# BVE-Reborn/rend3

Measured on NVIDIA H100. Metric: culled objects/s (fused frustum cull + object-uniform bake), higher is better.
Workload: dtype f32

## Files before the change

rend3_b200/csrc/r3_common.cuh:

```cuda
#pragma once
#include <cuda_runtime.h>
#include <stdint.h>

#include <string>
#include <vector>

#include "../../include/rend3_b200.h"

#define R3_EXPORT extern "C" __attribute__((visibility("default")))

constexpr int R3_MAX_CAMERAS = 64;

struct r3_iobuf {
    uint8_t* d = nullptr;
    uint64_t capacity_elements = 0, out_elems = 0, in_elems = 0, elem_size = 0;
    bool flipped = false, clear_on_swap = false, created = false;
    uint64_t out_off() const { return flipped ? capacity_elements / 2 : 0; }
    uint64_t in_off() const { return flipped ? 0 : capacity_elements / 2; }
};

struct r3_jobs {
    r3_batch_data* d_batches = nullptr; uint32_t batches_cap = 0, n_batches = 0;
    r3_region* d_regions = nullptr; uint32_t regions_cap = 0, n_regions = 0;
    uint32_t* d_region_first_inv = nullptr;
// ... 58 lines not shown
struct r3_anim_state;

struct r3_tri_record { float xyw[3][3]; uint32_t object_id; uint32_t vid[3]; uint32_t _pad[3]; };
static_assert(sizeof(r3_tri_record) == 64, "triangle record");

struct r3_ctx {
    int device = 0;
    cudaStream_t stream = nullptr;
    cudaStream_t side_stream = nullptr;
    std::string err;
    uint64_t launches = 0;
    bool coop_launch_ok = false;
    int sm_count = 1;
    r3_object* d_objects = nullptr; uint32_t n_slots = 0, objects_cap = 0; bool objects_borrowed = false;
    float4* d_hot_xyz = nullptr; float4* d_hot_w = nullptr; float4* d_hot_sphere = nullptr; uint32_t* d_enabled_bits = nullptr; uint32_t* d_affine_bits = nullptr;
    uint64_t hot_cap = 0; bool hot_valid = false;
    std::vector<uint64_t> sort_key; std::vector<uint8_t> sort_flags; std::vector<float> sort_loc;
    uint32_t* d_live_bits = nullptr; uint32_t live_bits_cap = 0; bool have_live = false;
    uint8_t* d_sort_key8 = nullptr; float* d_sort_loc = nullptr; uint32_t sort_dev_cap = 0; bool gpu_batching_ok = false;
    float4* d_mesh_spheres = nullptr; uint32_t n_mesh_spheres = 0, mesh_spheres_cap = 0;
    bool locations_moved = false;
    uint32_t sort_live_blend = 0, sort_wide_keys = 0;
    unsigned long long* d_gsort_keys[2] = {nullptr, nullptr}; uint64_t gsort_cap[2] = {0, 0}; uint32_t* d_gsort_hist = nullptr; uint64_t gsort_hist_cap = 0;
    uint32_t* d_gsort_header = nullptr; int gsort_src = 0; uint32_t gsort_n = 0; bool gsort_valid = false; float gsort_loc[3] = {0, 0, 0};
    uint64_t gsort_epoch = 0, gsort_sorted_epoch = ~0ull; uint32_t gsort_cameras_this_epoch = 0, gsort_cameras_last_epoch = 0;
    uint64_t max_total_invocations = 0, max_object_invocations = 0; bool max_invocations_valid = false;
    uint32_t* d_mesh = nullptr; uint64_t mesh_words = 0, mesh_cap = 0;
    r3_material* d_materials = nullptr; uint32_t n_materials = 0, materials_cap = 0;
    bool has_skybox = false; r3_texture_desc sky_desc{}; uint8_t* d_sky_texels = nullptr; uint64_t sky_cap = 0;
    r3_texture_desc* d_tex_descs = nullptr; uint32_t n_textures = 0, tex_descs_cap = 0; uint8_t* d_texels = nullptr; uint64_t texels_cap = 0, texel_bytes = 0;
// ... 67 lines not shown
template <typename T, typename C>
int r3_reserve_t(r3_ctx* c, T** ptr, C* cap, uint64_t need, bool keep = false, bool zero_new = false) {
    uint64_t cap64 = *cap;
    int rc = r3_reserve(c, (void**)ptr, &cap64, need, sizeof(T), keep, zero_new);
    *cap = (C)cap64;
    return rc;
}

int r3_launch_cull_bake(r3_ctx* c, r3_camera* cam, uint32_t mode);
int r3_launch_cull_bake_device_camera(r3_ctx* c, r3_camera* cam, uint32_t mode, const r3_camera_header* d_header);
int r3_camera_buffers(r3_ctx* c, r3_camera* cam, uint32_t mode);
int r3_split_objects(r3_ctx* c);
int r3_split_slots(r3_ctx* c, const uint32_t* d_slots, uint32_t n);
int r3_grow_hot(r3_ctx* c, uint32_t old_n, uint32_t n);
uint64_t r3_hot_capacity(uint64_t want);
int r3_launch_mask_word(r3_ctx* c, uint32_t* word_a, uint32_t* word_b, uint32_t keep_mask);
int r3_launch_triangle_cull(r3_ctx* c, r3_camera* cam);
int r3_host_batch_objects(r3_ctx* c, r3_camera* cam, const float vp_loc[3], uint32_t max_dispatch_count);
int r3_upload_jobs(r3_ctx* c, r3_camera* cam);
int r3_device_batch_objects(r3_ctx* c, r3_camera* cam, const float vp_loc[3], uint32_t max_dispatch_count);
int r3_download_jobs(r3_ctx* c, r3_camera* cam);
int r3_compute_max_invocations(r3_ctx* c);
void r3_new_frame_epoch(r3_ctx* c);
int r3_blend_collect(r3_ctx* c, bool* ran);
int r3_iobuf_new(r3_ctx* c, r3_iobuf* b, uint64_t elems, uint64_t elem_size, bool clear_on_swap);
int r3_iobuf_swap(r3_ctx* c, r3_iobuf* b, uint64_t new_elems);
int r3_launch_skinning(r3_ctx* c, const r3_skinning_input* d_inputs, const uint32_t* d_chunk_prefix, uint32_t n_skeletons, uint32_t total_chunks,
                       const float* d_joints, uint32_t n_joints);
void r3_anim_destroy(r3_ctx* c);
int r3_anim_stage_posed_locations(r3_ctx* c, bool* staged);
void r3_anim_apply_posed_locations(r3_ctx* c);
int r3_stage_moved_locations(r3_ctx* c, bool* staged);
int r3_grow_mesh_spheres(r3_ctx* c, uint32_t n);
int r3_reserve_point_buffer(r3_ctx* c, uint32_t n_lights);

#ifdef __CUDACC__
__device__ __forceinline__ uint32_t affine_w_bits(uint32_t j) { return j == 3 ? 0x3f800000u : 0u; }
__device__ __forceinline__ float mul_rn(float a, float b) { return __fmul_rn(a, b); }
__device__ __forceinline__ float add_rn(float a, float b) { return __fadd_rn(a, b); }
__device__ __forceinline__ float sub_rn(float a, float b) { return __fsub_rn(a, b); }
__device__ __forceinline__ float div_rn(float a, float b) { return __fdiv_rn(a, b); }
__device__ __forceinline__ float4 mat_vec_rn(const float* __restrict__ m, float x, float y, float z, float w) {
    float4 r;
    r.x = mul_rn(m[0], x); r.y = mul_rn(m[1], x); r.z = mul_rn(m[2], x); r.w = mul_rn(m[3], x);
    r.x = add_rn(r.x, mul_rn(m[4], y)); r.y = add_rn(r.y, mul_rn(m[5], y)); r.z = add_rn(r.z, mul_rn(m[6], y)); r.w = add_rn(r.w, mul_rn(m[7], y));
    r.x = add_rn(r.x, mul_rn(m[8], z)); r.y = add_rn(r.y, mul_rn(m[9], z)); r.z = add_rn(r.z, mul_rn(m[10], z)); r.w = add_rn(r.w, mul_rn(m[11], z));
    r.x = add_rn(r.x, mul_rn(m[12], w)); r.y = add_rn(r.y, mul_rn(m[13], w)); r.z = add_rn(r.z, mul_rn(m[14], w)); r.w = add_rn(r.w, mul_rn(m[15], w));
    return r;
}
__device__ __forceinline__ float4 mat_point_rn(const float* __restrict__ m, float x, float y, float z) {
    float4 r;
    r.x = mul_rn(m[0], x); r.y = mul_rn(m[1], x); r.z = mul_rn(m[2], x); r.w = mul_rn(m[3], x);
// ... 7 lines not shown
```

rend3_b200/csrc/r3_ctx.cu:

```cuda
#include <algorithm>
#include <cstdio>
#include <cstdlib>
#include <cstring>
#include <new>

#include "r3_common.cuh"

int r3_fail(r3_ctx* c, int code, const char* msg) {
    if (c) c->err = msg;
    return code;
}
int r3_cuda_fail(r3_ctx* c, cudaError_t e, const char* where) {
    if (c) {
        c->err = std::string(where) + ": " + cudaGetErrorString(e);
    }
    cudaGetLastError();
    return e == cudaErrorMemoryAllocation ? R3_E_OOM : R3_E_CUDA;
}

int r3_reserve(r3_ctx* c, void** ptr, uint64_t* cap, uint64_t need, size_t elem, bool keep, bool zero_new) {
    if (*ptr && *cap >= need) return R3_OK;
    uint64_t ncap = need < 16 ? 16 : need;
    void* n = nullptr;
    R3_CUDA(c, cudaMalloc(&n, ncap * elem));
// ... 38 lines not shown
    cudaMemsetAsync(c->d_point, 0, c->point_bytes_cap, c->stream);
    *out = c;
    return R3_OK;
}

static void free_jobs(r3_jobs& j) { cudaFree(j.d_batches); cudaFree(j.d_regions); cudaFree(j.d_region_first_inv); cudaFree(j.d_header); }

R3_EXPORT int r3_ctx_destroy(r3_ctx* c) {
    if (!c) return R3_E_INVALID;
    cudaSetDevice(c->device);
    r3_stream_sync(c);
    if (c->side_stream) cudaStreamSynchronize(c->side_stream);
    r3_peer_destroy(c);
    r3_anim_destroy(c);
    if (!c->objects_borrowed) cudaFree(c->d_objects);
    cudaFree(c->d_hot_xyz); cudaFree(c->d_hot_w); cudaFree(c->d_hot_sphere); cudaFree(c->d_enabled_bits); cudaFree(c->d_affine_bits); cudaFree(c->d_tex_descs); cudaFree(c->d_texels); cudaFree(c->d_sky_texels);
    cudaFree(c->d_sort_key8); cudaFree(c->d_sort_loc); cudaFree(c->d_gsort_keys[0]); cudaFree(c->d_gsort_keys[1]); cudaFree(c->d_gsort_hist); cudaFree(c->d_gsort_header);
    cudaFree(c->d_mesh_spheres); cudaFree(c->d_live_bits); cudaFree(c->d_mesh); cudaFree(c->d_materials); cudaFree(c->d_dir); cudaFree(c->d_point);
    cudaFree(c->d_light_mats); cudaFree(c->d_atlas); cudaFree(c->d_light_src); cudaFree(c->d_shadow_cams); cudaFree(c->d_point_src); cudaFree(c->d_point_live);
    for (auto& k : c->cams) {
        cudaFree(k.d_matrices); cudaFree(k.d_visible); cudaFree(k.d_visible_count); cudaFree(k.d_tile_state);
        if (k.d_gathered) {
            for (uint32_t r = 0; r < k.ex_ranks; ++r)
                if (k.ex_connected && r != k.ex_rank && k.ex_peers[r]) cudaIpcCloseMemHandle(k.ex_peers[r]);
            cudaFree(k.d_gathered);
        }
        cudaFree(k.d_ex_done); cudaFree(k.d_global_visible); cudaFree(k.d_merge_counts);
        for (int q = 0; q < R3_EXCHANGE_SLOTS; ++q) { if (k.ex_cull_done[q]) cudaEventDestroy(k.ex_cull_done[q]); if (k.ex_merge_done[q]) cudaEventDestroy(k.ex_merge_done[q]); }
        free_jobs(k.jobs[0]); free_jobs(k.jobs[1]);
        cudaFree(k.index_buffer.d); cudaFree(k.draw_call_buffer.d); cudaFree(k.results_buffer.d);
        cudaFree(k.d_resid_bits); cudaFree(k.d_word_scan); cudaFree(k.d_block_sums);
// ... 401 lines not shown
    if (n == c->n_slots) return R3_OK;
    cudaSetDevice(c->device);
    const uint32_t old_n = c->n_slots;
    if (n > c->objects_cap || !c->d_objects) R3_TRY(r3_reserve_t(c, &c->d_objects, &c->objects_cap, r3_hot_capacity(n), true));
    R3_CUDA(c, cudaMemsetAsync(c->d_objects + old_n, 0, (size_t)(n - old_n) * sizeof(r3_object), c->stream));
    R3_TRY(r3_grow_hot(c, old_n, n));
    R3_TRY(r3_grow_mesh_spheres(c, n));
    c->n_slots = n;
    const size_t sorted = c->sort_key.size();
    if (c->have_live && sorted < n) {
        c->sort_key.resize(n, 0); c->sort_flags.resize(n, 0); c->sort_loc.resize(3 * (size_t)n, 0.0f);
        const uint32_t old_words = (uint32_t)((sorted + 31) / 32), words = (n + 31) / 32;
        R3_TRY(r3_reserve_t(c, &c->d_live_bits, &c->live_bits_cap, words, true));
        const uint32_t whole = (sorted & 31u) ? old_words : (uint32_t)(sorted / 32);
        if (words > whole) R3_CUDA(c, cudaMemsetAsync(c->d_live_bits + whole, 0, (size_t)(words - whole) * 4, c->stream));
        if (sorted & 31u) R3_TRY(r3_launch_mask_word(c, c->d_live_bits + sorted / 32, nullptr, (1u << (sorted & 31u)) - 1u));
        if (n > c->sort_dev_cap || !c->d_sort_key8) {
            const uint32_t cap = (uint32_t)r3_hot_capacity(n);
            uint8_t* k8 = nullptr; float* l = nullptr;
            R3_CUDA(c, cudaMalloc((void**)&k8, cap));
            R3_CUDA(c, cudaMalloc((void**)&l, ((size_t)cap * 3 + 4) * 4));
            if (sorted) {
                R3_CUDA(c, cudaMemcpyAsync(k8, c->d_sort_key8, sorted, cudaMemcpyDeviceToDevice, c->stream));
                R3_CUDA(c, cudaMemcpyAsync(l, c->d_sort_loc, sorted * 12, cudaMemcpyDeviceToDevice, c->stream));
            }
            R3_CUDA(c, r3_stream_sync(c));
            cudaFree(c->d_sort_key8); cudaFree(c->d_sort_loc);
            c->d_sort_key8 = k8; c->d_sort_loc = l; c->sort_dev_cap = cap;
        }
        R3_CUDA(c, cudaMemsetAsync(c->d_sort_key8 + sorted, 0, n - sorted, c->stream));
        R3_CUDA(c, cudaMemsetAsync(c->d_sort_loc + 3 * sorted, 0, (n - sorted) * 12, c->stream));
// ... 290 lines not shown
```

rend3_b200/csrc/r3_cull_bake.cu:

```cuda
#include <cstdlib>
#include <type_traits>

#include "r3_common.cuh"
#include "r3_scan.cuh"

namespace {

constexpr int CB_THREADS = 256;
constexpr int CB_WARPS = CB_THREADS / 32;
constexpr int CB_WT = 4;
constexpr int CB_CTA_OBJECTS = CB_WARPS * CB_WT * 32;
constexpr int CP_THREADS = 1024;
constexpr int CP_OBJECTS = CP_THREADS * 32;
constexpr int CP_CTAS_PER_TILE = CP_OBJECTS / CB_CTA_OBJECTS;

struct CullBakeParams {
    float view[16];
    float view_proj[16];
    float frustum[5][4];
    uint32_t object_count;
};
struct DeviceCameraParams {
    const r3_camera_header* cam;
    uint32_t object_count;
};
constexpr int CAM_FLOATS = 52;

__global__ void __launch_bounds__(256) split_objects_kernel(const float4* __restrict__ objects, uint32_t n, float* __restrict__ rows_xyz, float* __restrict__ rows_w,
                                                            float4* __restrict__ spheres, uint32_t* __restrict__ enabled_bits, uint32_t* __restrict__ affine_bits) {
    const int lane = threadIdx.x & 31, k = lane & 7, g = lane >> 3;
    const uint32_t wtile = (blockIdx.x * blockDim.x + threadIdx.x) >> 5, base = wtile * 32u;
    if (base >= n) return;
    uint32_t bits = 0, abits = 0;
#pragma unroll
    for (int it = 0; it < 8; ++it) {
        const uint32_t obj = base + it * 4 + g;
        float4 r = make_float4(0.f, 0.f, 0.f, 0.f);
        if (obj < n) {
            r = __ldcs(&objects[(size_t)obj * 8 + k]);
            if (k < 4) {
                float* xyz = rows_xyz + (size_t)obj * 12 + k;
                xyz[0] = r.x; xyz[4] = r.y; xyz[8] = r.z;
                rows_w[(size_t)obj * 4 + k] = r.w;
            } else if (k == 4) spheres[obj] = r;
        }
        const uint32_t b = __ballot_sync(0xFFFFFFFFu, k == 7 && obj < n && __float_as_uint(r.y) != 0u);
        bits |= (((b >> 7) & 1u) | (((b >> 15) & 1u) << 1) | (((b >> 23) & 1u) << 2) | (((b >> 31) & 1u) << 3)) << (it * 4);
        const uint32_t a = __ballot_sync(0xFFFFFFFFu, k < 4 && obj < n && __float_as_uint(r.w) == affine_w_bits(k));
#pragma unroll
        for (int q = 0; q < 4; ++q) abits |= (((a >> (8 * q)) & 0xFu) == 0xFu ? 1u : 0u) << (it * 4 + q);
    }
    if (lane == 0) { enabled_bits[wtile] = bits; affine_bits[wtile] = abits; }
}
__global__ void __launch_bounds__(256) split_slots_kernel(const float4* __restrict__ objects, const uint32_t* __restrict__ slots, uint32_t n_updates, uint32_t n_slots,
                                                          float* __restrict__ rows_xyz, float* __restrict__ rows_w, float4* __restrict__ spheres,
                                                          uint32_t* __restrict__ enabled_bits, uint32_t* __restrict__ affine_bits) {
    const uint32_t i = (blockIdx.x * blockDim.x + threadIdx.x) >> 3, k = threadIdx.x & 7;
    const uint32_t s = i < n_updates ? slots[i] : n_slots;
    const bool ok = s < n_slots;
    float4 r = make_float4(0.f, 0.f, 0.f, 0.f);
    if (ok) {
        r = objects[(size_t)s * 8 + k];
        if (k < 4) {
            float* xyz = rows_xyz + (size_t)s * 12 + k;
            xyz[0] = r.x; xyz[4] = r.y; xyz[8] = r.z;
            rows_w[(size_t)s * 4 + k] = r.w;
        } else if (k == 4) spheres[s] = r;
    }
    const uint32_t a = __ballot_sync(0xFFFFFFFFu, ok && k < 4 && __float_as_uint(r.w) == affine_w_bits(k));
    if (ok && k == 7) {
        const uint32_t bit = 1u << (s & 31u);
        if (__float_as_uint(r.y) != 0u) atomicOr(&enabled_bits[s >> 5], bit);
        else atomicAnd(&enabled_bits[s >> 5], ~bit);
        if (((a >> (threadIdx.x & 24u)) & 0xFu) == 0xFu) atomicOr(&affine_bits[s >> 5], bit);
        else atomicAnd(&affine_bits[s >> 5], ~bit);
    }
}

template <bool BAKE, bool CULL, bool LIVE, typename Params = CullBakeParams>
__global__ void __launch_bounds__(CB_THREADS)
cull_bake_kernel(const float4* __restrict__ rows_xyz, const float* __restrict__ rows_w, const uint32_t* __restrict__ affine_bits, const float4* __restrict__ spheres,
                 const uint32_t* __restrict__ enabled_bits, const uint32_t* __restrict__ live_bits, float4* __restrict__ matrices, uint32_t* __restrict__ words,
                 uint32_t* __restrict__ cta_counts, const __grid_constant__ Params p) {
    __shared__ uint32_t s_count[CB_WARPS];
    __shared__ float4 s_rows[BAKE ? CB_WARPS : 1][96];
    const int lane = threadIdx.x & 31, warp = threadIdx.x >> 5;
    const float* view;
    const float* view_proj;
    const float* frustum;
    if constexpr (std::is_same<Params, DeviceCameraParams>::value) {
        __shared__ float s_cam[CAM_FLOATS];
        const float* src = reinterpret_cast<const float*>(p.cam);
        if (threadIdx.x < CAM_FLOATS) s_cam[threadIdx.x] = __ldg(src + (threadIdx.x < 32 ? threadIdx.x : threadIdx.x + 4));
        __syncthreads();
        view = s_cam; view_proj = s_cam + 16; frustum = s_cam + 32;
    } else {
        view = p.view; view_proj = p.view_proj; frustum = &p.frustum[0][0];
    }
    const int col = lane & 3, sub = lane >> 2;
    uint32_t count = 0;
#pragma unroll 2
    for (int wt = 0; wt < CB_WT; ++wt) {
        const uint32_t wtile = (blockIdx.x * CB_WARPS + warp) * CB_WT + wt;
        const uint32_t base = wtile * 32u;
        if (base >= p.object_count) break;
        float4 t[3];
        float4 sp = make_float4(0.f, 0.f, 0.f, 0.f);
        uint32_t enabled = 0u, affine = 0u;
        if (BAKE) {
#pragma unroll
            for (int q = 0; q < 3; ++q) {
                const uint32_t e = q * 32 + lane;
                t[q] = base + e / 3u < p.object_count ? __ldcs(&rows_xyz[(size_t)base * 3 + e]) : make_float4(0.f, 0.f, 0.f, 0.f);
            }
        }
        if (CULL && base + lane < p.object_count) sp = __ldcs(&spheres[base + lane]);
        if (BAKE || (CULL && !LIVE)) enabled = __ldg(&enabled_bits[wtile]);
        if (BAKE) affine = __ldg(&affine_bits[wtile]);
        if (BAKE) {
            float4* tile = s_rows[warp];
            __syncwarp();
#pragma unroll
            for (int q = 0; q < 3; ++q) tile[q * 32 + lane] = t[q];
            __syncwarp();
            const float* tf = reinterpret_cast<const float*>(tile);
#pragma unroll
            for (int it = 0; it < 4; ++it) {
                const uint32_t slot = it * 8 + sub, obj = base + slot;
                if (obj < p.object_count && ((enabled >> slot) & 1u)) {
                    const float* c = tf + slot * 12 + col;
                    const float w = ((affine >> slot) & 1u) ? (col == 3 ? 1.0f : 0.0f) : __ldcs(&rows_w[(size_t)obj * 4 + col]);
                    float4* dst = &matrices[(size_t)obj * 8 + col];
                    __stcs(dst, mat_vec_rn(view, c[0], c[4], c[8], w));
                    __stcs(dst + 4, mat_vec_rn(view_proj, c[0], c[4], c[8], w));
                }
            }
        }
        if (CULL) {
            const uint32_t live = LIVE ? __ldg(&live_bits[wtile]) : enabled;
            const float neg_radius = -sp.w;
            bool inside = true;
#pragma unroll
            for (int pl = 0; pl < 5; ++pl) {
                const float* f = frustum + 4 * pl;
                const float d = add_rn(add_rn(add_rn(mul_rn(f[0], sp.x), mul_rn(f[1], sp.y)), mul_rn(f[2], sp.z)), f[3]);
                inside = inside && (d >= neg_radius);
            }
            const uint32_t word = __ballot_sync(0xFFFFFFFFu, base + lane < p.object_count && ((live >> lane) & 1u) && inside);
            if (lane == 0) words[wtile] = word;
            count += __popc(word);
        }
    }
    if (CULL) {
        if (lane == 0) s_count[warp] = count;
// ... 137 lines not shown
    memcpy(p.view_proj, cam->header.view_proj, 64);
    memcpy(p.frustum, cam->header.frustum, 80);
    p.object_count = n;
    const uint32_t n_ctas = (n + CB_CTA_OBJECTS - 1) / CB_CTA_OBJECTS, n_words = (n + 31) / 32;
    const uint64_t set_words = (((uint64_t)n_words + n_ctas + 63) / 64) * 64;
    R3_TRY(r3_reserve_t(c, &cam->d_tile_state, &cam->tile_state_cap, set_words + 2));
    if (cull) cam->words_set ^= 1u;
    uint32_t* words = reinterpret_cast<uint32_t*>(cam->d_tile_state) + (size_t)cam->words_set * set_words;
    cam->d_words = words;
    uint32_t* cta_counts = words + n_words;
    if (!c->hot_valid) return r3_fail(c, R3_E_STATE, "object_uniform_upload before set_objects");
    float4* mats = reinterpret_cast<float4*>(cam->d_matrices);
    const bool live = c->have_live && cull && c->sort_flags.size() >= (size_t)n;
#define R3_CB_LAUNCH(B, C, L) \
    cull_bake_kernel<B, C, L><<<n_ctas, CB_THREADS, 0, c->stream>>>(c->d_hot_xyz, reinterpret_cast<const float*>(c->d_hot_w), c->d_affine_bits, c->d_hot_sphere, \
                                                                    c->d_enabled_bits, c->d_live_bits, mats, words, cta_counts, p)
    r3_stage_begin(c, R3_STAGE_CULL_BAKE);
    if (d_header) {
        const DeviceCameraParams dp{d_header, n};
        const uint32_t* live_bits = live ? c->d_live_bits : c->d_enabled_bits;
#define R3_CB_DEV_LAUNCH(B, C)                                                                                                                       \
    cull_bake_kernel<B, C, C, DeviceCameraParams><<<n_ctas, CB_THREADS, 0, c->stream>>>(c->d_hot_xyz, reinterpret_cast<const float*>(c->d_hot_w),     \
                                                                                      c->d_affine_bits, c->d_hot_sphere, c->d_enabled_bits, live_bits, \
                                                                                      mats, words, cta_counts, dp)
        if (bake && cull) R3_CB_DEV_LAUNCH(true, true);
        else if (bake) R3_CB_DEV_LAUNCH(true, false);
        else R3_CB_DEV_LAUNCH(false, true);
#undef R3_CB_DEV_LAUNCH
    } else if (bake && cull) { if (live) R3_CB_LAUNCH(true, true, true); else R3_CB_LAUNCH(true, true, false); }
    else if (bake) R3_CB_LAUNCH(true, false, false);
    else { if (live) R3_CB_LAUNCH(false, true, true); else R3_CB_LAUNCH(false, true, false); }
#undef R3_CB_LAUNCH
    r3_stage_end(c);
    R3_CHECK_LAUNCH(c, "cull_bake_kernel");
    if (cull) {
        const uint32_t n_tiles = (n_words + CP_THREADS - 1) / CP_THREADS;
        ExchangeParams ex{};
        if (cam->ex_connected) {
// ... 24 lines not shown
int r3_launch_cull_bake_device_camera(r3_ctx* c, r3_camera* cam, uint32_t mode, const r3_camera_header* d_header) {
    return launch_cull_bake(c, cam, mode, d_header);
}

uint64_t r3_hot_capacity(uint64_t want) {
    uint64_t cap = 1024;
    while (cap < want) cap *= 2;
    if (cap > want + want / 8 && want > (1u << 20)) cap = want + want / 8;
    return cap;
}
int r3_split_objects(r3_ctx* c) {
    const uint32_t n = c->n_slots;
    const uint64_t want = n ? n : 1;
    if (want > c->hot_cap) {
        cudaFree(c->d_hot_xyz); cudaFree(c->d_hot_w); cudaFree(c->d_hot_sphere); cudaFree(c->d_enabled_bits); cudaFree(c->d_affine_bits);
        c->d_hot_xyz = nullptr; c->d_hot_w = nullptr; c->d_hot_sphere = nullptr; c->d_enabled_bits = nullptr; c->d_affine_bits = nullptr; c->hot_cap = 0;
        const uint64_t cap = r3_hot_capacity(want);
        R3_CUDA(c, cudaMalloc((void**)&c->d_hot_xyz, cap * 48));
        R3_CUDA(c, cudaMalloc((void**)&c->d_hot_w, cap * 16));
        R3_CUDA(c, cudaMalloc((void**)&c->d_hot_sphere, cap * 16));
        R3_CUDA(c, cudaMalloc((void**)&c->d_enabled_bits, ((cap + 31) / 32 + 1) * 4));
        R3_CUDA(c, cudaMalloc((void**)&c->d_affine_bits, ((cap + 31) / 32 + 1) * 4));
        c->hot_cap = cap;
    }
    if (n) {
        const uint32_t warps = (n + 31) / 32;
        split_objects_kernel<<<(warps + 7) / 8, 256, 0, c->stream>>>(reinterpret_cast<const float4*>(c->d_objects), n, reinterpret_cast<float*>(c->d_hot_xyz),
                                                                      reinterpret_cast<float*>(c->d_hot_w), c->d_hot_sphere, c->d_enabled_bits, c->d_affine_bits);
        R3_CHECK_LAUNCH(c, "split_objects_kernel");
    }
    c->hot_valid = true;
    return R3_OK;
}
int r3_split_slots(r3_ctx* c, const uint32_t* d_slots, uint32_t n) {
    if (!c->hot_valid || n == 0) return R3_OK;
    split_slots_kernel<<<(n * 8 + 255) / 256, 256, 0, c->stream>>>(reinterpret_cast<const float4*>(c->d_objects), d_slots, n, c->n_slots,
                                                                    reinterpret_cast<float*>(c->d_hot_xyz), reinterpret_cast<float*>(c->d_hot_w), c->d_hot_sphere,
                                                                    c->d_enabled_bits, c->d_affine_bits);
    R3_CHECK_LAUNCH(c, "split_slots_kernel");
    return R3_OK;
}
namespace {
__global__ void mask_word_kernel(uint32_t* word_a, uint32_t* word_b, uint32_t keep_mask) {
    if (word_a) *word_a &= keep_mask;
    if (word_b) *word_b &= keep_mask;
}
}
int r3_launch_mask_word(r3_ctx* c, uint32_t* word_a, uint32_t* word_b, uint32_t keep_mask) {
    mask_word_kernel<<<1, 1, 0, c->stream>>>(word_a, word_b, keep_mask);
    R3_CHECK_LAUNCH(c, "mask_word_kernel");
    return R3_OK;
}
int r3_grow_hot(r3_ctx* c, uint32_t old_n, uint32_t n) {
    if (!c->hot_valid) old_n = 0;
    const uint64_t old_words = ((uint64_t)old_n + 31) / 32;
    if ((uint64_t)n > c->hot_cap || !c->d_hot_xyz) {
        const uint64_t cap = r3_hot_capacity(n ? n : 1), bit_words = (cap + 31) / 32 + 1;
        float4 *xyz = nullptr, *w = nullptr, *sph = nullptr;
        uint32_t *en = nullptr, *af = nullptr;
        R3_CUDA(c, cudaMalloc((void**)&xyz, cap * 48));
        R3_CUDA(c, cudaMalloc((void**)&w, cap * 16));
        R3_CUDA(c, cudaMalloc((void**)&sph, cap * 16));
        R3_CUDA(c, cudaMalloc((void**)&en, bit_words * 4));
        R3_CUDA(c, cudaMalloc((void**)&af, bit_words * 4));
        if (old_n) {
            R3_CUDA(c, cudaMemcpyAsync(xyz, c->d_hot_xyz, (size_t)old_n * 48, cudaMemcpyDeviceToDevice, c->stream));
            R3_CUDA(c, cudaMemcpyAsync(w, c->d_hot_w, (size_t)old_n * 16, cudaMemcpyDeviceToDevice, c->stream));
            R3_CUDA(c, cudaMemcpyAsync(sph, c->d_hot_sphere, (size_t)old_n * 16, cudaMemcpyDeviceToDevice, c->stream));
            R3_CUDA(c, cudaMemcpyAsync(en, c->d_enabled_bits, old_words * 4, cudaMemcpyDeviceToDevice, c->stream));
            R3_CUDA(c, cudaMemcpyAsync(af, c->d_affine_bits, old_words * 4, cudaMemcpyDeviceToDevice, c->stream));
        }
        R3_CUDA(c, r3_stream_sync(c));
        cudaFree(c->d_hot_xyz); cudaFree(c->d_hot_w); cudaFree(c->d_hot_sphere); cudaFree(c->d_enabled_bits); cudaFree(c->d_affine_bits);
        c->d_hot_xyz = xyz; c->d_hot_w = w; c->d_hot_sphere = sph; c->d_enabled_bits = en; c->d_affine_bits = af; c->hot_cap = cap;
    }
    const uint64_t first_word = old_n / 32, new_words = ((uint64_t)n + 31) / 32;
    if (n > old_n) {
        R3_CUDA(c, cudaMemsetAsync(c->d_hot_xyz + (size_t)old_n * 3, 0, (size_t)(n - old_n) * 48, c->stream));
        R3_CUDA(c, cudaMemsetAsync(c->d_hot_w + old_n, 0, (size_t)(n - old_n) * 16, c->stream));
        R3_CUDA(c, cudaMemsetAsync(c->d_hot_sphere + old_n, 0, (size_t)(n - old_n) * 16, c->stream));
    }
    const uint64_t whole = (old_n & 31u) ? first_word + 1 : first_word;
    if (new_words > whole) {
        R3_CUDA(c, cudaMemsetAsync(c->d_enabled_bits + whole, 0, (new_words - whole) * 4, c->stream));
        R3_CUDA(c, cudaMemsetAsync(c->d_affine_bits + whole, 0, (new_words - whole) * 4, c->stream));
    }
    if (old_n & 31u) R3_TRY(r3_launch_mask_word(c, c->d_enabled_bits + first_word, c->d_affine_bits + first_word, (1u << (old_n & 31u)) - 1u));
    c->hot_valid = true;
    return R3_OK;
}

R3_EXPORT int r3_exchange_create(r3_ctx* c, uint32_t camera, uint32_t n_ranks, uint32_t my_rank, uint32_t max_objects_per_rank, uint8_t handle_out[R3_IPC_HANDLE_BYTES]) {
    if (!c || !handle_out) return r3_fail(c, R3_E_INVALID, "exchange_create: null");
    if (n_ranks == 0 || n_ranks > R3_MAX_EXCHANGE_RANKS || my_rank >= n_ranks || max_objects_per_rank == 0) return r3_fail(c, R3_E_INVALID, "exchange_create: bad rank layout");
    r3_camera* cam = r3_get_camera(c, camera);
    if (!cam) return r3_fail(c, R3_E_INVALID, "exchange_create: bad camera");
    static_assert(sizeof(cudaIpcMemHandle_t) == R3_IPC_HANDLE_BYTES, "IPC handle size");
    cudaSetDevice(c->device);
    if (cam->d_gathered) return r3_fail(c, R3_E_STATE, "exchange_create: already created for this camera");
    const uint32_t wpr = (((max_objects_per_rank + 31u) / 32u) + 63u) & ~63u;
    const size_t total_words = EX_HEADER_WORDS + (size_t)EX_SLOTS * n_ranks * wpr;
    R3_CUDA(c, cudaMalloc((void**)&cam->d_gathered, total_words * 4));
// ... 143 lines not shown
```

rend3_b200/csrc/r3_object_transforms.cu:

```cuda
#include <cstring>
#include <vector>

#include "r3_common.cuh"

namespace {

constexpr uint32_t OT_THREADS = 256;

template <bool SPARSE>
__global__ void __launch_bounds__(OT_THREADS, 4)
object_transforms_kernel(const float4* __restrict__ mats, const uint32_t* __restrict__ slots, uint32_t n, uint32_t n_slots, const float4* __restrict__ mesh_spheres,
                         float4* __restrict__ objects, float* __restrict__ rows_xyz, float* __restrict__ rows_w, float4* __restrict__ spheres,
                         uint32_t* __restrict__ affine_bits, float* __restrict__ sort_loc, uint32_t sort_n) {
    const uint32_t lane = threadIdx.x & 31u, k = lane & 3u, g = lane >> 2, first = lane & ~3u;
    const uint32_t wtile = (blockIdx.x * blockDim.x + threadIdx.x) >> 5, base = wtile * 32u;
    if (base >= n) return;
    uint32_t abits = 0;
#pragma unroll
    for (uint32_t it = 0; it < 4; ++it) {
        const uint32_t i = base + it * 8u + g;
        uint32_t s = n_slots;
        if (i < n) s = SPARSE ? __ldg(slots + i) : i;
        const bool ok = s < n_slots;
        float4 col = make_float4(0.f, 0.f, 0.f, 0.f), ms = col;
        if (ok) { col = __ldcs(&mats[(size_t)i * 4 + k]); ms = __ldg(&mesh_spheres[s]); }
        float x[4], y[4], z[4];
#pragma unroll
        for (uint32_t j = 0; j < 4; ++j) {
            x[j] = __shfl_sync(0xFFFFFFFFu, col.x, first + j); y[j] = __shfl_sync(0xFFFFFFFFu, col.y, first + j); z[j] = __shfl_sync(0xFFFFFFFFu, col.z, first + j);
        }
        const uint32_t a = __ballot_sync(0xFFFFFFFFu, ok && __float_as_uint(col.w) == affine_w_bits(k));
        const bool affine = ((a >> first) & 0xFu) == 0xFu;
        if (!SPARSE) {
#pragma unroll
            for (uint32_t q = 0; q < 8; ++q) abits |= (((a >> (4u * q)) & 0xFu) == 0xFu ? 1u : 0u) << (it * 8u + q);
        }
        if (ok) {
            float ls[3];
#pragma unroll
            for (int c = 0; c < 3; ++c) ls[c] = add_rn(add_rn(mul_rn(x[c], x[c]), mul_rn(y[c], y[c])), mul_rn(z[c], z[c]));
            const float max_scale = __fsqrt_rn(fmaxf(ls[0], fmaxf(ls[1], ls[2])));
            float4 sph;
            sph.x = add_rn(add_rn(add_rn(mul_rn(x[0], ms.x), mul_rn(x[1], ms.y)), mul_rn(x[2], ms.z)), mul_rn(x[3], 1.0f));
            sph.y = add_rn(add_rn(add_rn(mul_rn(y[0], ms.x), mul_rn(y[1], ms.y)), mul_rn(y[2], ms.z)), mul_rn(y[3], 1.0f));
            sph.z = add_rn(add_rn(add_rn(mul_rn(z[0], ms.x), mul_rn(z[1], ms.y)), mul_rn(z[2], ms.z)), mul_rn(z[3], 1.0f));
            sph.w = mul_rn(max_scale, ms.w);
            objects[(size_t)s * 8 + k] = col;
            float* xyz = rows_xyz + (size_t)s * 12 + k;
            xyz[0] = col.x; xyz[4] = col.y; xyz[8] = col.z;
            rows_w[(size_t)s * 4 + k] = col.w;
            if (k == 0) objects[(size_t)s * 8 + 4] = sph;
            else if (k == 1) spheres[s] = sph;
            else if (k == 2) {
                if (sort_loc && s < sort_n) {
                    float* l = sort_loc + 3 * (size_t)s;
                    l[0] = add_rn(x[3], add_rn(add_rn(mul_rn(x[0], 0.0f), mul_rn(x[1], 0.0f)), mul_rn(x[2], 0.0f)));
                    l[1] = add_rn(y[3], add_rn(add_rn(mul_rn(y[0], 0.0f), mul_rn(y[1], 0.0f)), mul_rn(y[2], 0.0f)));
                    l[2] = add_rn(z[3], add_rn(add_rn(mul_rn(z[0], 0.0f), mul_rn(z[1], 0.0f)), mul_rn(z[2], 0.0f)));
                }
            } else if (SPARSE) {
                const uint32_t bit = 1u << (s & 31u);
                if (affine) atomicOr(&affine_bits[s >> 5], bit);
                else atomicAnd(&affine_bits[s >> 5], ~bit);
            }
        }
    }
    if (!SPARSE && lane == 0) {
        if (n - base >= 32u) affine_bits[wtile] = abits;
        else {
            const uint32_t mask = (1u << (n - base)) - 1u;
            atomicAnd(&affine_bits[wtile], ~mask | abits);
            atomicOr(&affine_bits[wtile], abits);
        }
    }
}

__global__ void scatter_mesh_spheres_kernel(const float4* __restrict__ src, const uint32_t* __restrict__ slots, uint32_t n, float4* __restrict__ dst) {
    const uint32_t i = blockIdx.x * blockDim.x + threadIdx.x;
    if (i < n) dst[slots[i]] = src[i];
}

int check_slots(r3_ctx* c, const uint32_t* slots, uint32_t n, uint32_t limit, const char* beyond, const char* twice) {
    std::vector<uint64_t> seen(((size_t)limit + 63) / 64, 0ull);
    for (uint32_t i = 0; i < n; ++i) {
        const uint32_t s = slots[i];
        if (s >= limit) return r3_fail(c, R3_E_INVALID, beyond);
        const uint64_t bit = 1ull << (s & 63u);
// ... 3 lines not shown
    return R3_OK;
}

int check_state(r3_ctx* c) {
    if (!c->d_objects || !c->hot_valid) return r3_fail(c, R3_E_STATE, "set_object_transforms before set_objects");
    if (c->n_mesh_spheres < c->n_slots) return r3_fail(c, R3_E_STATE, "set_object_transforms: r3_set_object_mesh_spheres does not cover every slot");
    if (c->objects_borrowed) return r3_fail(c, R3_E_STATE, "set_object_transforms: the object buffer is borrowed (r3_set_objects_device)");
    return R3_OK;
}

int launch_transforms(r3_ctx* c, const uint32_t* d_slots, const float* d_mats, uint32_t n) {
    const uint32_t sort_n = c->have_live ? (uint32_t)c->sort_key.size() : 0u;
    const uint32_t ctas = (uint32_t)(((uint64_t)n + OT_THREADS - 1) / OT_THREADS);
    auto kernel = d_slots ? object_transforms_kernel<true> : object_transforms_kernel<false>;
    kernel<<<ctas, OT_THREADS, 0, c->stream>>>(reinterpret_cast<const float4*>(d_mats), d_slots, n, c->n_slots, c->d_mesh_spheres, reinterpret_cast<float4*>(c->d_objects),
                                               reinterpret_cast<float*>(c->d_hot_xyz), reinterpret_cast<float*>(c->d_hot_w), c->d_hot_sphere, c->d_affine_bits,
                                               sort_n ? c->d_sort_loc : nullptr, sort_n);
    R3_CHECK_LAUNCH(c, "object_transforms_kernel");
    r3_new_frame_epoch(c);
    if (sort_n) c->locations_moved = true;
    return R3_OK;
}

}

R3_EXPORT int r3_set_object_mesh_spheres(r3_ctx* c, const uint32_t* slots, const float* center_radius, uint32_t n) {
    if (!c) return R3_E_INVALID;
    if (!center_radius && n) return r3_fail(c, R3_E_INVALID, "set_object_mesh_spheres: null");
    cudaSetDevice(c->device);
    if (!slots) {
        R3_TRY(r3_reserve_t(c, &c->d_mesh_spheres, &c->mesh_spheres_cap, n));
        if (n) R3_CUDA(c, cudaMemcpyAsync(c->d_mesh_spheres, center_radius, (size_t)n * 16, cudaMemcpyHostToDevice, c->stream));
// ... 64 lines not shown
```

Baseline: 14.04 billion.

## Read only radius when sphere centre equals translation in fused cull-bake

Adds a per-object bitmask marking objects whose bounding-sphere centre is bit-identical to the transform's translation column, plus a compact radius array. When baking and culling together, the kernel loads just the 4-byte radius for those objects and takes the centre from the transform rows already staged in shared memory, instead of loading the full 16-byte sphere. This aims to cut global memory traffic in the bandwidth-bound cull pass. In exchange, the split, transform and grow paths must maintain two extra buffers and bitmask updates, and each tile does one more bitmask load.

```diff
diff --git a/rend3_b200/csrc/r3_common.cuh b/rend3_b200/csrc/r3_common.cuh
--- a/rend3_b200/csrc/r3_common.cuh
+++ b/rend3_b200/csrc/r3_common.cuh
@@ -96,6 +96,7 @@
     int sm_count = 1;
     r3_object* d_objects = nullptr; uint32_t n_slots = 0, objects_cap = 0; bool objects_borrowed = false;
     float4* d_hot_xyz = nullptr; float4* d_hot_w = nullptr; float4* d_hot_sphere = nullptr; uint32_t* d_enabled_bits = nullptr; uint32_t* d_affine_bits = nullptr;
+    float* d_hot_radius = nullptr; uint32_t* d_centre_bits = nullptr;
     uint64_t hot_cap = 0; bool hot_valid = false;
     std::vector<uint64_t> sort_key; std::vector<uint8_t> sort_flags; std::vector<float> sort_loc;
     uint32_t* d_live_bits = nullptr; uint32_t live_bits_cap = 0; bool have_live = false;
@@ -193,7 +194,7 @@
 int r3_split_slots(r3_ctx* c, const uint32_t* d_slots, uint32_t n);
 int r3_grow_hot(r3_ctx* c, uint32_t old_n, uint32_t n);
 uint64_t r3_hot_capacity(uint64_t want);
-int r3_launch_mask_word(r3_ctx* c, uint32_t* word_a, uint32_t* word_b, uint32_t keep_mask);
+int r3_launch_mask_word(r3_ctx* c, uint32_t* word_a, uint32_t* word_b, uint32_t* word_c, uint32_t keep_mask);
 int r3_launch_triangle_cull(r3_ctx* c, r3_camera* cam);
 int r3_host_batch_objects(r3_ctx* c, r3_camera* cam, const float vp_loc[3], uint32_t max_dispatch_count);
 int r3_upload_jobs(r3_ctx* c, r3_camera* cam);
@@ -215,6 +216,9 @@
 
 #ifdef __CUDACC__
 __device__ __forceinline__ uint32_t affine_w_bits(uint32_t j) { return j == 3 ? 0x3f800000u : 0u; }
+__device__ __forceinline__ bool centre_is_translation(float cx, float cy, float cz, float tx, float ty, float tz) {
+    return __float_as_uint(cx) == __float_as_uint(tx) && __float_as_uint(cy) == __float_as_uint(ty) && __float_as_uint(cz) == __float_as_uint(tz);
+}
 __device__ __forceinline__ float mul_rn(float a, float b) { return __fmul_rn(a, b); }
 __device__ __forceinline__ float add_rn(float a, float b) { return __fadd_rn(a, b); }
 __device__ __forceinline__ float sub_rn(float a, float b) { return __fsub_rn(a, b); }
diff --git a/rend3_b200/csrc/r3_ctx.cu b/rend3_b200/csrc/r3_ctx.cu
--- a/rend3_b200/csrc/r3_ctx.cu
+++ b/rend3_b200/csrc/r3_ctx.cu
@@ -76,7 +76,7 @@
     r3_peer_destroy(c);
     r3_anim_destroy(c);
     if (!c->objects_borrowed) cudaFree(c->d_objects);
-    cudaFree(c->d_hot_xyz); cudaFree(c->d_hot_w); cudaFree(c->d_hot_sphere); cudaFree(c->d_enabled_bits); cudaFree(c->d_affine_bits); cudaFree(c->d_tex_descs); cudaFree(c->d_texels); cudaFree(c->d_sky_texels);
+    cudaFree(c->d_hot_xyz); cudaFree(c->d_hot_w); cudaFree(c->d_hot_sphere); cudaFree(c->d_enabled_bits); cudaFree(c->d_affine_bits); cudaFree(c->d_hot_radius); cudaFree(c->d_centre_bits); cudaFree(c->d_tex_descs); cudaFree(c->d_texels); cudaFree(c->d_sky_texels);
     cudaFree(c->d_sort_key8); cudaFree(c->d_sort_loc); cudaFree(c->d_gsort_keys[0]); cudaFree(c->d_gsort_keys[1]); cudaFree(c->d_gsort_hist); cudaFree(c->d_gsort_header);
     cudaFree(c->d_mesh_spheres); cudaFree(c->d_live_bits); cudaFree(c->d_mesh); cudaFree(c->d_materials); cudaFree(c->d_dir); cudaFree(c->d_point);
     cudaFree(c->d_light_mats); cudaFree(c->d_atlas); cudaFree(c->d_light_src); cudaFree(c->d_shadow_cams); cudaFree(c->d_point_src); cudaFree(c->d_point_live);
@@ -508,7 +508,7 @@
         R3_TRY(r3_reserve_t(c, &c->d_live_bits, &c->live_bits_cap, words, true));
         const uint32_t whole = (sorted & 31u) ? old_words : (uint32_t)(sorted / 32);
         if (words > whole) R3_CUDA(c, cudaMemsetAsync(c->d_live_bits + whole, 0, (size_t)(words - whole) * 4, c->stream));
-        if (sorted & 31u) R3_TRY(r3_launch_mask_word(c, c->d_live_bits + sorted / 32, nullptr, (1u << (sorted & 31u)) - 1u));
+        if (sorted & 31u) R3_TRY(r3_launch_mask_word(c, c->d_live_bits + sorted / 32, nullptr, nullptr, (1u << (sorted & 31u)) - 1u));
         if (n > c->sort_dev_cap || !c->d_sort_key8) {
             const uint32_t cap = (uint32_t)r3_hot_capacity(n);
             uint8_t* k8 = nullptr; float* l = nullptr;
diff --git a/rend3_b200/csrc/r3_cull_bake.cu b/rend3_b200/csrc/r3_cull_bake.cu
--- a/rend3_b200/csrc/r3_cull_bake.cu
+++ b/rend3_b200/csrc/r3_cull_bake.cu
@@ -27,11 +27,12 @@
 constexpr int CAM_FLOATS = 52;
 
 __global__ void __launch_bounds__(256) split_objects_kernel(const float4* __restrict__ objects, uint32_t n, float* __restrict__ rows_xyz, float* __restrict__ rows_w,
-                                                            float4* __restrict__ spheres, uint32_t* __restrict__ enabled_bits, uint32_t* __restrict__ affine_bits) {
+                                                            float4* __restrict__ spheres, float* __restrict__ radii, uint32_t* __restrict__ enabled_bits,
+                                                            uint32_t* __restrict__ affine_bits, uint32_t* __restrict__ centre_bits) {
     const int lane = threadIdx.x & 31, k = lane & 7, g = lane >> 3;
     const uint32_t wtile = (blockIdx.x * blockDim.x + threadIdx.x) >> 5, base = wtile * 32u;
     if (base >= n) return;
-    uint32_t bits = 0, abits = 0;
+    uint32_t bits = 0, abits = 0, cbits = 0;
 #pragma unroll
     for (int it = 0; it < 8; ++it) {
         const uint32_t obj = base + it * 4 + g;
@@ -42,19 +43,22 @@
                 float* xyz = rows_xyz + (size_t)obj * 12 + k;
                 xyz[0] = r.x; xyz[4] = r.y; xyz[8] = r.z;
                 rows_w[(size_t)obj * 4 + k] = r.w;
-            } else if (k == 4) spheres[obj] = r;
+            } else if (k == 4) { spheres[obj] = r; radii[obj] = r.w; }
         }
         const uint32_t b = __ballot_sync(0xFFFFFFFFu, k == 7 && obj < n && __float_as_uint(r.y) != 0u);
         bits |= (((b >> 7) & 1u) | (((b >> 15) & 1u) << 1) | (((b >> 23) & 1u) << 2) | (((b >> 31) & 1u) << 3)) << (it * 4);
         const uint32_t a = __ballot_sync(0xFFFFFFFFu, k < 4 && obj < n && __float_as_uint(r.w) == affine_w_bits(k));
 #pragma unroll
         for (int q = 0; q < 4; ++q) abits |= (((a >> (8 * q)) & 0xFu) == 0xFu ? 1u : 0u) << (it * 4 + q);
-    }
-    if (lane == 0) { enabled_bits[wtile] = bits; affine_bits[wtile] = abits; }
+        const float tx = __shfl_up_sync(0xFFFFFFFFu, r.x, 1), ty = __shfl_up_sync(0xFFFFFFFFu, r.y, 1), tz = __shfl_up_sync(0xFFFFFFFFu, r.z, 1);
+        const uint32_t cb = __ballot_sync(0xFFFFFFFFu, k == 4 && obj < n && centre_is_translation(r.x, r.y, r.z, tx, ty, tz));
+        cbits |= (((cb >> 4) & 1u) | (((cb >> 12) & 1u) << 1) | (((cb >> 20) & 1u) << 2) | (((cb >> 28) & 1u) << 3)) << (it * 4);
+    }
+    if (lane == 0) { enabled_bits[wtile] = bits; affine_bits[wtile] = abits; centre_bits[wtile] = cbits; }
 }
 __global__ void __launch_bounds__(256) split_slots_kernel(const float4* __restrict__ objects, const uint32_t* __restrict__ slots, uint32_t n_updates, uint32_t n_slots,
-                                                          float* __restrict__ rows_xyz, float* __restrict__ rows_w, float4* __restrict__ spheres,
-                                                          uint32_t* __restrict__ enabled_bits, uint32_t* __restrict__ affine_bits) {
+                                                          float* __restrict__ rows_xyz, float* __restrict__ rows_w, float4* __restrict__ spheres, float* __restrict__ radii,
+                                                          uint32_t* __restrict__ enabled_bits, uint32_t* __restrict__ affine_bits, uint32_t* __restrict__ centre_bits) {
     const uint32_t i = (blockIdx.x * blockDim.x + threadIdx.x) >> 3, k = threadIdx.x & 7;
     const uint32_t s = i < n_updates ? slots[i] : n_slots;
     const bool ok = s < n_slots;
@@ -65,22 +69,26 @@
             float* xyz = rows_xyz + (size_t)s * 12 + k;
             xyz[0] = r.x; xyz[4] = r.y; xyz[8] = r.z;
             rows_w[(size_t)s * 4 + k] = r.w;
-        } else if (k == 4) spheres[s] = r;
+        } else if (k == 4) { spheres[s] = r; radii[s] = r.w; }
     }
     const uint32_t a = __ballot_sync(0xFFFFFFFFu, ok && k < 4 && __float_as_uint(r.w) == affine_w_bits(k));
+    const float tx = __shfl_up_sync(0xFFFFFFFFu, r.x, 1), ty = __shfl_up_sync(0xFFFFFFFFu, r.y, 1), tz = __shfl_up_sync(0xFFFFFFFFu, r.z, 1);
+    const uint32_t cb = __ballot_sync(0xFFFFFFFFu, ok && k == 4 && centre_is_translation(r.x, r.y, r.z, tx, ty, tz));
     if (ok && k == 7) {
         const uint32_t bit = 1u << (s & 31u);
         if (__float_as_uint(r.y) != 0u) atomicOr(&enabled_bits[s >> 5], bit);
         else atomicAnd(&enabled_bits[s >> 5], ~bit);
         if (((a >> (threadIdx.x & 24u)) & 0xFu) == 0xFu) atomicOr(&affine_bits[s >> 5], bit);
         else atomicAnd(&affine_bits[s >> 5], ~bit);
+        if ((cb >> ((threadIdx.x & 24u) + 4u)) & 1u) atomicOr(&centre_bits[s >> 5], bit);
+        else atomicAnd(&centre_bits[s >> 5], ~bit);
     }
 }
 
 template <bool BAKE, bool CULL, bool LIVE, typename Params = CullBakeParams>
 __global__ void __launch_bounds__(CB_THREADS)
 cull_bake_kernel(const float4* __restrict__ rows_xyz, const float* __restrict__ rows_w, const uint32_t* __restrict__ affine_bits, const float4* __restrict__ spheres,
-                 const uint32_t* __restrict__ enabled_bits, const uint32_t* __restrict__ live_bits, float4* __restrict__ matrices, uint32_t* __restrict__ words,
+                 const float* __restrict__ radii, const uint32_t* __restrict__ centre_bits, const uint32_t* __restrict__ enabled_bits, const uint32_t* __restrict__ live_bits, float4* __restrict__ matrices, uint32_t* __restrict__ words,
                  uint32_t* __restrict__ cta_counts, const __grid_constant__ Params p) {
     __shared__ uint32_t s_count[CB_WARPS];
     __shared__ float4 s_rows[BAKE ? CB_WARPS : 1][96];
@@ -106,7 +114,8 @@
         if (base >= p.object_count) break;
         float4 t[3];
         float4 sp = make_float4(0.f, 0.f, 0.f, 0.f);
-        uint32_t enabled = 0u, affine = 0u;
+        uint32_t enabled = 0u, affine = 0u, centred = 0u;
+        if (BAKE && CULL) centred = __ldg(&centre_bits[wtile]);
         if (BAKE) {
 #pragma unroll
             for (int q = 0; q < 3; ++q) {
@@ -114,7 +123,11 @@
                 t[q] = base + e / 3u < p.object_count ? __ldcs(&rows_xyz[(size_t)base * 3 + e]) : make_float4(0.f, 0.f, 0.f, 0.f);
             }
         }
-        if (CULL && base + lane < p.object_count) sp = __ldcs(&spheres[base + lane]);
+        const bool centre_from_tile = BAKE && CULL && ((centred >> lane) & 1u);
+        if (CULL && base + lane < p.object_count) {
+            if (centre_from_tile) sp.w = __ldcs(&radii[base + lane]);
+            else sp = __ldcs(&spheres[base + lane]);
+        }
         if (BAKE || (CULL && !LIVE)) enabled = __ldg(&enabled_bits[wtile]);
         if (BAKE) affine = __ldg(&affine_bits[wtile]);
         if (BAKE) {
@@ -138,6 +151,12 @@
         }
         if (CULL) {
             const uint32_t live = LIVE ? __ldg(&live_bits[wtile]) : enabled;
+            if constexpr (BAKE) {
+                if (centre_from_tile) {
+                    const float* tr = reinterpret_cast<const float*>(s_rows[warp]) + lane * 12 + 3;
+                    sp.x = tr[0]; sp.y = tr[4]; sp.z = tr[8];
+                }
+            }
             const float neg_radius = -sp.w;
             bool inside = true;
 #pragma unroll
@@ -305,14 +324,15 @@
     const bool live = c->have_live && cull && c->sort_flags.size() >= (size_t)n;
 #define R3_CB_LAUNCH(B, C, L) \
     cull_bake_kernel<B, C, L><<<n_ctas, CB_THREADS, 0, c->stream>>>(c->d_hot_xyz, reinterpret_cast<const float*>(c->d_hot_w), c->d_affine_bits, c->d_hot_sphere, \
-                                                                    c->d_enabled_bits, c->d_live_bits, mats, words, cta_counts, p)
+                                                                    c->d_hot_radius, c->d_centre_bits, c->d_enabled_bits, c->d_live_bits, mats, words, cta_counts, p)
     r3_stage_begin(c, R3_STAGE_CULL_BAKE);
     if (d_header) {
         const DeviceCameraParams dp{d_header, n};
         const uint32_t* live_bits = live ? c->d_live_bits : c->d_enabled_bits;
 #define R3_CB_DEV_LAUNCH(B, C)                                                                                                                       \
     cull_bake_kernel<B, C, C, DeviceCameraParams><<<n_ctas, CB_THREADS, 0, c->stream>>>(c->d_hot_xyz, reinterpret_cast<const float*>(c->d_hot_w),     \
-                                                                                      c->d_affine_bits, c->d_hot_sphere, c->d_enabled_bits, live_bits, \
+                                                                                      c->d_affine_bits, c->d_hot_sphere, c->d_hot_radius, c->d_centre_bits, \
+                                                                                      c->d_enabled_bits, live_bits, \
                                                                                       mats, words, cta_counts, dp)
         if (bake && cull) R3_CB_DEV_LAUNCH(true, true);
         else if (bake) R3_CB_DEV_LAUNCH(true, false);
@@ -367,19 +387,24 @@
     const uint64_t want = n ? n : 1;
     if (want > c->hot_cap) {
         cudaFree(c->d_hot_xyz); cudaFree(c->d_hot_w); cudaFree(c->d_hot_sphere); cudaFree(c->d_enabled_bits); cudaFree(c->d_affine_bits);
-        c->d_hot_xyz = nullptr; c->d_hot_w = nullptr; c->d_hot_sphere = nullptr; c->d_enabled_bits = nullptr; c->d_affine_bits = nullptr; c->hot_cap = 0;
+        cudaFree(c->d_hot_radius); cudaFree(c->d_centre_bits);
+        c->d_hot_xyz = nullptr; c->d_hot_w = nullptr; c->d_hot_sphere = nullptr; c->d_enabled_bits = nullptr; c->d_affine_bits = nullptr;
+        c->d_hot_radius = nullptr; c->d_centre_bits = nullptr; c->hot_cap = 0;
         const uint64_t cap = r3_hot_capacity(want);
         R3_CUDA(c, cudaMalloc((void**)&c->d_hot_xyz, cap * 48));
         R3_CUDA(c, cudaMalloc((void**)&c->d_hot_w, cap * 16));
         R3_CUDA(c, cudaMalloc((void**)&c->d_hot_sphere, cap * 16));
+        R3_CUDA(c, cudaMalloc((void**)&c->d_hot_radius, cap * 4));
         R3_CUDA(c, cudaMalloc((void**)&c->d_enabled_bits, ((cap + 31) / 32 + 1) * 4));
         R3_CUDA(c, cudaMalloc((void**)&c->d_affine_bits, ((cap + 31) / 32 + 1) * 4));
+        R3_CUDA(c, cudaMalloc((void**)&c->d_centre_bits, ((cap + 31) / 32 + 1) * 4));
         c->hot_cap = cap;
     }
     if (n) {
         const uint32_t warps = (n + 31) / 32;
         split_objects_kernel<<<(warps + 7) / 8, 256, 0, c->stream>>>(reinterpret_cast<const float4*>(c->d_objects), n, reinterpret_cast<float*>(c->d_hot_xyz),
-                                                                      reinterpret_cast<float*>(c->d_hot_w), c->d_hot_sphere, c->d_enabled_bits, c->d_affine_bits);
+                                                                      reinterpret_cast<float*>(c->d_hot_w), c->d_hot_sphere, c->d_hot_radius, c->d_enabled_bits,
+                                                                      c->d_affine_bits, c->d_centre_bits);
         R3_CHECK_LAUNCH(c, "split_objects_kernel");
     }
     c->hot_valid = true;
@@ -389,18 +414,19 @@
     if (!c->hot_valid || n == 0) return R3_OK;
     split_slots_kernel<<<(n * 8 + 255) / 256, 256, 0, c->stream>>>(reinterpret_cast<const float4*>(c->d_objects), d_slots, n, c->n_slots,
                                                                     reinterpret_cast<float*>(c->d_hot_xyz), reinterpret_cast<float*>(c->d_hot_w), c->d_hot_sphere,
-                                                                    c->d_enabled_bits, c->d_affine_bits);
+                                                                    c->d_hot_radius, c->d_enabled_bits, c->d_affine_bits, c->d_centre_bits);
     R3_CHECK_LAUNCH(c, "split_slots_kernel");
     return R3_OK;
 }
 namespace {
-__global__ void mask_word_kernel(uint32_t* word_a, uint32_t* word_b, uint32_t keep_mask) {
+__global__ void mask_word_kernel(uint32_t* word_a, uint32_t* word_b, uint32_t* word_c, uint32_t keep_mask) {
     if (word_a) *word_a &= keep_mask;
     if (word_b) *word_b &= keep_mask;
-}
-}
-int r3_launch_mask_word(r3_ctx* c, uint32_t* word_a, uint32_t* word_b, uint32_t keep_mask) {
-    mask_word_kernel<<<1, 1, 0, c->stream>>>(word_a, word_b, keep_mask);
+    if (word_c) *word_c &= keep_mask;
+}
+}
+int r3_launch_mask_word(r3_ctx* c, uint32_t* word_a, uint32_t* word_b, uint32_t* word_c, uint32_t keep_mask) {
+    mask_word_kernel<<<1, 1, 0, c->stream>>>(word_a, word_b, word_c, keep_mask);
     R3_CHECK_LAUNCH(c, "mask_word_kernel");
     return R3_OK;
 }
@@ -410,35 +436,45 @@
     if ((uint64_t)n > c->hot_cap || !c->d_hot_xyz) {
         const uint64_t cap = r3_hot_capacity(n ? n : 1), bit_words = (cap + 31) / 32 + 1;
         float4 *xyz = nullptr, *w = nullptr, *sph = nullptr;
-        uint32_t *en = nullptr, *af = nullptr;
+        float* rad = nullptr;
+        uint32_t *en = nullptr, *af = nullptr, *ce = nullptr;
         R3_CUDA(c, cudaMalloc((void**)&xyz, cap * 48));
         R3_CUDA(c, cudaMalloc((void**)&w, cap * 16));
         R3_CUDA(c, cudaMalloc((void**)&sph, cap * 16));
+        R3_CUDA(c, cudaMalloc((void**)&rad, cap * 4));
         R3_CUDA(c, cudaMalloc((void**)&en, bit_words * 4));
         R3_CUDA(c, cudaMalloc((void**)&af, bit_words * 4));
+        R3_CUDA(c, cudaMalloc((void**)&ce, bit_words * 4));
         if (old_n) {
             R3_CUDA(c, cudaMemcpyAsync(xyz, c->d_hot_xyz, (size_t)old_n * 48, cudaMemcpyDeviceToDevice, c->stream));
             R3_CUDA(c, cudaMemcpyAsync(w, c->d_hot_w, (size_t)old_n * 16, cudaMemcpyDeviceToDevice, c->stream));
             R3_CUDA(c, cudaMemcpyAsync(sph, c->d_hot_sphere, (size_t)old_n * 16, cudaMemcpyDeviceToDevice, c->stream));
+            R3_CUDA(c, cudaMemcpyAsync(rad, c->d_hot_radius, (size_t)old_n * 4, cudaMemcpyDeviceToDevice, c->stream));
             R3_CUDA(c, cudaMemcpyAsync(en, c->d_enabled_bits, old_words * 4, cudaMemcpyDeviceToDevice, c->stream));
             R3_CUDA(c, cudaMemcpyAsync(af, c->d_affine_bits, old_words * 4, cudaMemcpyDeviceToDevice, c->stream));
+            R3_CUDA(c, cudaMemcpyAsync(ce, c->d_centre_bits, old_words * 4, cudaMemcpyDeviceToDevice, c->stream));
         }
         R3_CUDA(c, r3_stream_sync(c));
         cudaFree(c->d_hot_xyz); cudaFree(c->d_hot_w); cudaFree(c->d_hot_sphere); cudaFree(c->d_enabled_bits); cudaFree(c->d_affine_bits);
+        cudaFree(c->d_hot_radius); cudaFree(c->d_centre_bits);
         c->d_hot_xyz = xyz; c->d_hot_w = w; c->d_hot_sphere = sph; c->d_enabled_bits = en; c->d_affine_bits = af; c->hot_cap = cap;
+        c->d_hot_radius = rad; c->d_centre_bits = ce;
     }
     const uint64_t first_word = old_n / 32, new_words = ((uint64_t)n + 31) / 32;
     if (n > old_n) {
         R3_CUDA(c, cudaMemsetAsync(c->d_hot_xyz + (size_t)old_n * 3, 0, (size_t)(n - old_n) * 48, c->stream));
         R3_CUDA(c, cudaMemsetAsync(c->d_hot_w + old_n, 0, (size_t)(n - old_n) * 16, c->stream));
         R3_CUDA(c, cudaMemsetAsync(c->d_hot_sphere + old_n, 0, (size_t)(n - old_n) * 16, c->stream));
+        R3_CUDA(c, cudaMemsetAsync(c->d_hot_radius + old_n, 0, (size_t)(n - old_n) * 4, c->stream));
     }
     const uint64_t whole = (old_n & 31u) ? first_word + 1 : first_word;
     if (new_words > whole) {
         R3_CUDA(c, cudaMemsetAsync(c->d_enabled_bits + whole, 0, (new_words - whole) * 4, c->stream));
         R3_CUDA(c, cudaMemsetAsync(c->d_affine_bits + whole, 0, (new_words - whole) * 4, c->stream));
-    }
-    if (old_n & 31u) R3_TRY(r3_launch_mask_word(c, c->d_enabled_bits + first_word, c->d_affine_bits + first_word, (1u << (old_n & 31u)) - 1u));
+        R3_CUDA(c, cudaMemsetAsync(c->d_centre_bits + whole, 0, (new_words - whole) * 4, c->stream));
+    }
+    if (old_n & 31u)
+        R3_TRY(r3_launch_mask_word(c, c->d_enabled_bits + first_word, c->d_affine_bits + first_word, c->d_centre_bits + first_word, (1u << (old_n & 31u)) - 1u));
     c->hot_valid = true;
     return R3_OK;
 }
diff --git a/rend3_b200/csrc/r3_object_transforms.cu b/rend3_b200/csrc/r3_object_transforms.cu
--- a/rend3_b200/csrc/r3_object_transforms.cu
+++ b/rend3_b200/csrc/r3_object_transforms.cu
@@ -11,11 +11,12 @@
 __global__ void __launch_bounds__(OT_THREADS, 4)
 object_transforms_kernel(const float4* __restrict__ mats, const uint32_t* __restrict__ slots, uint32_t n, uint32_t n_slots, const float4* __restrict__ mesh_spheres,
                          float4* __restrict__ objects, float* __restrict__ rows_xyz, float* __restrict__ rows_w, float4* __restrict__ spheres,
-                         uint32_t* __restrict__ affine_bits, float* __restrict__ sort_loc, uint32_t sort_n) {
+                         float* __restrict__ radii, uint32_t* __restrict__ affine_bits, uint32_t* __restrict__ centre_bits, float* __restrict__ sort_loc,
+                         uint32_t sort_n) {
     const uint32_t lane = threadIdx.x & 31u, k = lane & 3u, g = lane >> 2, first = lane & ~3u;
     const uint32_t wtile = (blockIdx.x * blockDim.x + threadIdx.x) >> 5, base = wtile * 32u;
     if (base >= n) return;
-    uint32_t abits = 0;
+    uint32_t abits = 0, cbits = 0;
 #pragma unroll
     for (uint32_t it = 0; it < 4; ++it) {
         const uint32_t i = base + it * 8u + g;
@@ -31,26 +32,31 @@
         }
         const uint32_t a = __ballot_sync(0xFFFFFFFFu, ok && __float_as_uint(col.w) == affine_w_bits(k));
         const bool affine = ((a >> first) & 0xFu) == 0xFu;
+        float ls[3];
+#pragma unroll
+        for (int c = 0; c < 3; ++c) ls[c] = add_rn(add_rn(mul_rn(x[c], x[c]), mul_rn(y[c], y[c])), mul_rn(z[c], z[c]));
+        const float max_scale = __fsqrt_rn(fmaxf(ls[0], fmaxf(ls[1], ls[2])));
+        float4 sph;
+        sph.x = add_rn(add_rn(add_rn(mul_rn(x[0], ms.x), mul_rn(x[1], ms.y)), mul_rn(x[2], ms.z)), mul_rn(x[3], 1.0f));
+        sph.y = add_rn(add_rn(add_rn(mul_rn(y[0], ms.x), mul_rn(y[1], ms.y)), mul_rn(y[2], ms.z)), mul_rn(y[3], 1.0f));
+        sph.z = add_rn(add_rn(add_rn(mul_rn(z[0], ms.x), mul_rn(z[1], ms.y)), mul_rn(z[2], ms.z)), mul_rn(z[3], 1.0f));
+        sph.w = mul_rn(max_scale, ms.w);
+        const uint32_t cb = __ballot_sync(0xFFFFFFFFu, ok && centre_is_translation(sph.x, sph.y, sph.z, x[3], y[3], z[3]));
+        const bool centred = (cb >> first) & 1u;
         if (!SPARSE) {
 #pragma unroll
-            for (uint32_t q = 0; q < 8; ++q) abits |= (((a >> (4u * q)) & 0xFu) == 0xFu ? 1u : 0u) << (it * 8u + q);
+            for (uint32_t q = 0; q < 8; ++q) {
+                abits |= (((a >> (4u * q)) & 0xFu) == 0xFu ? 1u : 0u) << (it * 8u + q);
+                cbits |= ((cb >> (4u * q)) & 1u) << (it * 8u + q);
+            }
         }
         if (ok) {
-            float ls[3];
-#pragma unroll
-            for (int c = 0; c < 3; ++c) ls[c] = add_rn(add_rn(mul_rn(x[c], x[c]), mul_rn(y[c], y[c])), mul_rn(z[c], z[c]));
-            const float max_scale = __fsqrt_rn(fmaxf(ls[0], fmaxf(ls[1], ls[2])));
-            float4 sph;
-            sph.x = add_rn(add_rn(add_rn(mul_rn(x[0], ms.x), mul_rn(x[1], ms.y)), mul_rn(x[2], ms.z)), mul_rn(x[3], 1.0f));
-            sph.y = add_rn(add_rn(add_rn(mul_rn(y[0], ms.x), mul_rn(y[1], ms.y)), mul_rn(y[2], ms.z)), mul_rn(y[3], 1.0f));
-            sph.z = add_rn(add_rn(add_rn(mul_rn(z[0], ms.x), mul_rn(z[1], ms.y)), mul_rn(z[2], ms.z)), mul_rn(z[3], 1.0f));
-            sph.w = mul_rn(max_scale, ms.w);
             objects[(size_t)s * 8 + k] = col;
             float* xyz = rows_xyz + (size_t)s * 12 + k;
             xyz[0] = col.x; xyz[4] = col.y; xyz[8] = col.z;
             rows_w[(size_t)s * 4 + k] = col.w;
             if (k == 0) objects[(size_t)s * 8 + 4] = sph;
-            else if (k == 1) spheres[s] = sph;
+            else if (k == 1) { spheres[s] = sph; radii[s] = sph.w; }
             else if (k == 2) {
                 if (sort_loc && s < sort_n) {
                     float* l = sort_loc + 3 * (size_t)s;
@@ -62,15 +68,19 @@
                 const uint32_t bit = 1u << (s & 31u);
                 if (affine) atomicOr(&affine_bits[s >> 5], bit);
                 else atomicAnd(&affine_bits[s >> 5], ~bit);
+                if (centred) atomicOr(&centre_bits[s >> 5], bit);
+                else atomicAnd(&centre_bits[s >> 5], ~bit);
             }
         }
     }
     if (!SPARSE && lane == 0) {
-        if (n - base >= 32u) affine_bits[wtile] = abits;
+        if (n - base >= 32u) { affine_bits[wtile] = abits; centre_bits[wtile] = cbits; }
         else {
             const uint32_t mask = (1u << (n - base)) - 1u;
             atomicAnd(&affine_bits[wtile], ~mask | abits);
             atomicOr(&affine_bits[wtile], abits);
+            atomicAnd(&centre_bits[wtile], ~mask | cbits);
+            atomicOr(&centre_bits[wtile], cbits);
         }
     }
 }
@@ -104,8 +114,8 @@
     const uint32_t ctas = (uint32_t)(((uint64_t)n + OT_THREADS - 1) / OT_THREADS);
     auto kernel = d_slots ? object_transforms_kernel<true> : object_transforms_kernel<false>;
     kernel<<<ctas, OT_THREADS, 0, c->stream>>>(reinterpret_cast<const float4*>(d_mats), d_slots, n, c->n_slots, c->d_mesh_spheres, reinterpret_cast<float4*>(c->d_objects),
-                                               reinterpret_cast<float*>(c->d_hot_xyz), reinterpret_cast<float*>(c->d_hot_w), c->d_hot_sphere, c->d_affine_bits,
-                                               sort_n ? c->d_sort_loc : nullptr, sort_n);
+                                               reinterpret_cast<float*>(c->d_hot_xyz), reinterpret_cast<float*>(c->d_hot_w), c->d_hot_sphere, c->d_hot_radius,
+                                               c->d_affine_bits, c->d_centre_bits, sort_n ? c->d_sort_loc : nullptr, sort_n);
     R3_CHECK_LAUNCH(c, "object_transforms_kernel");
     r3_new_frame_epoch(c);
     if (sort_n) c->locations_moved = true;
```

Result: faster. 14.86 billion, median of 6 (+5.9%).
